# naver/deep-image-retrieval

Measured on AMD Instinct MI355X. Metric: images/sec descriptor extraction (resnet101-GeM, 1024x1024), higher is better.
Workload: dtype fp16p

## Files before the change

### deep-image-retrieval_amd/csrc/conv_igemm.hip

```cpp
#include "dir_common.h"
#include "conv_device.h"
#include "conv_igemm.h"

#include <stdlib.h>
#include <string.h>
#include <algorithm>

namespace dir {

template <class DT, int BM, int BN, int WGM, int WGN, int NST, int BK, bool CIN16, bool SPLITK>
__global__ void __launch_bounds__(64 * WGM * WGN) conv_igemm_kernel(const ConvArgs a) {
    static_assert(NST >= 2 && NST <= 8, "ring depth");
    static_assert((BK == 64 || BK == 32) && (!CIN16 || BK == 64), "K-step");
    constexpr int RB = BK * 2;
    constexpr int CPR = BK / 8;
    constexpr int KS = BK / 16;
    constexpr int NT = 64 * WGM * WGN;
    constexpr int TM = BM / WGM / 32;
    constexpr int TN = BN / WGN / 32;
    constexpr int NA = BM * CPR / NT;
    constexpr int NB = BN * CPR / NT;
    constexpr int LPS = NA + NB;
    static_assert(TM >= 1 && TN >= 1, "wave tile");
    static_assert(NA >= 1 && NB >= 1 && (BM * CPR) % NT == 0 && (BN * CPR) % NT == 0, "chunk split");
// ... 508 lines not shown
        (long)ceil_div(a.M, 64) * (a.Cout / 128) >= 96)
        return prev;
    return last;
}

int conv_pick_dual_variant(const ConvArgs& a, bool any_size) {
    const bool ok = a.x2 && a.R == 1 && a.S == 1 && a.stride == 1 && a.pad == 0 && a.H == a.OH && a.W == a.OW &&
                    a.Cin % 64 == 0 && a.Cin2 % 64 == 0 && a.res == nullptr && a.ksplit <= 1;
    if (!ok) return -1;
    {
        const int v = find_variant("64x256_wregd1x1");
        if (v >= 0 && !env().no_wregd && conv1x1_wregd_admissible(a) &&
            (any_size || (long)ceil_div(a.M, 64) * (a.Cout / 256) >= 1024))
            return v;
    }
    if (a.Cout % 256 != 0 || (!any_size && (long)ceil_div(a.M, 256) * (a.Cout / 256) < 192)) return -1;
    if (env().lc1x1) {
        const int vl = find_variant("256x256_lc1x1");
        if (vl >= 0 && conv1x1_lc_admissible(a)) return vl;
    }
    const int v = find_variant("256x256_persist1x1_x3");
    if (v < 0 || kVariants[v].launch_dual == nullptr) return -1;
    return v;
}

template <class DT>
__global__ void conv_splitk_finalize_kernel(const float* __restrict__ partial, const float* __restrict__ bias,
                                            const uint16_t* res, uint16_t* y,
                                            long total8, int Cout, long MC, int ksplit, int relu, int* ovf_flag) {
    const long i8 = (long)blockIdx.x * blockDim.x + threadIdx.x;
    if (i8 >= total8) return;
    const long o = i8 * 8;
    const int n = (int)(o % Cout);
    float v[8];
    const f32x4_t b0 = *(const DIR_GLOBAL f32x4_t*)(bias + n), b1 = *(const DIR_GLOBAL f32x4_t*)(bias + n + 4);
#pragma unroll
    for (int e = 0; e < 4; ++e) v[e] = b0[e], v[4 + e] = b1[e];
    for (int z = 0; z < ksplit; ++z) {
        const float* p = partial + (size_t)z * MC + o;
        const f32x4_t p0 = *(const DIR_GLOBAL f32x4_t*)p, p1 = *(const DIR_GLOBAL f32x4_t*)(p + 4);
#pragma unroll
        for (int e = 0; e < 4; ++e) v[e] += p0[e], v[4 + e] += p1[e];
    }
    if (res) {
        const u32x4_t rv = gload16(res + o);
#pragma unroll
        for (int e = 0; e < 4; ++e) {
            float lo, hi;
            DT::unpack(rv[e], lo, hi);
            v[2 * e] += lo;
            v[2 * e + 1] += hi;
        }
    }
    if (relu) relu8(v);
    const u32x4_t ov = pack8<DT>(v);
    gstore16(y + o, ov);
    Ovf<DT> ovf;
    ovf.see(ov);
    ovf.flush(ovf_flag);
}

size_t conv_splitk_bytes(const ConvArgs& a, int ksplit) {
    return ksplit > 1 ? (size_t)ksplit * a.M * a.Cout * sizeof(float) : 0;
}

int conv_splitk_factor(int v, const ConvArgs& a) {
    if (v < 0 || v >= kNumVariants || !kVariants[v].has_splitk || a.Cin == 16) return 1;
    const ConvVariant& cv = kVariants[v];
    const long tiles = (long)ceil_div(a.M, cv.BM) * (a.Cout / cv.BN);
    const int T = a.Ktot / cv.BK;
    if (tiles > 160 || T < 8) return 1;
    int s = (int)std::min<long>(std::min<long>(8, 512 / tiles), T / 4);
    while (s > 1 && conv_splitk_bytes(a, s) > kSplitKMaxBytes) --s;
    return s < 2 ? 1 : s;
}

int conv_launch(const ConvArgs& a, int dtype, int variant, hipStream_t stream) {
    if (a.Cout % 64 != 0) return fail(DIR_ERR_INVALID, "conv: Cout must be a multiple of 64");
    const bool cin16 = (a.Cin == 16);
    if (cin16) {
        if (a.R != 4 || a.S != 4 || a.stride != 1)
            return fail(DIR_ERR_INVALID, "conv: Cin == 16 is only the 4x4 s1 space-to-depth stem");
    } else if (a.Cin % 64 != 0) {
        return fail(DIR_ERR_INVALID, "conv: Cin must be a multiple of 64 (or 16 for the stem)");
    }
    if (a.R > 4 || a.S > 4) return fail(DIR_ERR_INVALID, "conv: filter larger than 4x4");
    if ((long)a.B * a.H * a.W * a.Cin >= (1L << 30) || (long)a.M * a.Cout >= (1L << 30) ||
        (long)a.Cout * a.Ktot >= (1L << 30))
        return fail(DIR_ERR_INVALID, "conv: tensor exceeds 2^31 bytes; lower the batch");
    if (((uintptr_t)a.x & 15) || ((uintptr_t)a.w & 15) || ((uintptr_t)a.y & 15) ||
        ((uintptr_t)a.res & 15) || ((uintptr_t)a.bias & 15))
        return fail(DIR_ERR_INVALID, "conv: tensors must be 16-byte aligned");
    if (dtype != DIR_BF16 && dtype != DIR_FP16) return fail(DIR_ERR_INVALID, "conv: bad dtype");
    if (a.x2) {
        if (variant < 0) variant = conv_pick_dual_variant(a);
        if (variant < 0 || variant >= kNumVariants || kVariants[variant].launch_dual == nullptr ||
            !kVariants[variant].admissible_dual(a) || a.R != 1 || a.S != 1 || a.stride != 1 || a.res || a.ksplit > 1 ||
            a.Cin2 % 64 != 0 || a.Ktot != a.Cin + a.Cin2 || ((uintptr_t)a.x2 & 15) ||
            (long)a.B * a.H2 * a.W2 * a.Cin2 >= (1L << 30))
            return fail(DIR_ERR_INVALID, "conv: no two-source form for this shape / variant");
        hipError_t e = kVariants[variant].launch_dual(a, dtype, stream);
        if (e != hipSuccess)
            return fail(DIR_ERR_HIP, std::string("conv launch ") + kVariants[variant].name + "/dual: " + hipGetErrorString(e));
        return DIR_OK;
    }
    if (variant < 0) variant = conv_pick_variant(a);
    if (!conv_variant_admissible(variant, a))
        return fail(DIR_ERR_INVALID, "conv: variant not admissible for this shape");
    const ConvVariant& cv = kVariants[variant];
    if (a.ksplit > 1) {
        if (!cv.has_splitk || cin16)
            return fail(DIR_ERR_INVALID, "conv: this variant has no split-K form");
        if (!a.partial || ((uintptr_t)a.partial & 15))
            return fail(DIR_ERR_INVALID, "conv: split-K needs a 16-byte aligned fp32 scratch buffer");
        if (a.ksplit > a.Ktot / cv.BK) return fail(DIR_ERR_INVALID, "conv: more K slices than K-steps");
    }
    hipError_t e = cv.launch(a, dtype, stream);
    if (e != hipSuccess)
        return fail(DIR_ERR_HIP, std::string("conv launch ") + cv.name + ": " + hipGetErrorString(e));
    if (a.ksplit > 1) {
        const long MC = (long)a.M * a.Cout, total8 = MC / 8;
        const dim3 grid((unsigned)((total8 + 255) / 256));
        if (dtype == DIR_BF16)
            hipLaunchKernelGGL(conv_splitk_finalize_kernel<BF16>, grid, dim3(256), 0, stream, a.partial, a.bias,
                               a.res, a.y, total8, a.Cout, MC, a.ksplit, a.relu, a.ovf);
        else
            hipLaunchKernelGGL(conv_splitk_finalize_kernel<FP16>, grid, dim3(256), 0, stream, a.partial, a.bias,
                               a.res, a.y, total8, a.Cout, MC, a.ksplit, a.relu, a.ovf);
        e = hipGetLastError();
        if (e != hipSuccess) return fail(DIR_ERR_HIP, std::string("conv split-K finalize: ") + hipGetErrorString(e));
    }
    return DIR_OK;
}

template <class DT>
__global__ void conv_naive_kernel(const ConvArgs a) {
    const long idx = (long)blockIdx.x * blockDim.x + threadIdx.x;
    if (idx >= (long)a.M * a.Cout) return;
    const int n = (int)(idx % a.Cout);
    const int m = (int)(idx / a.Cout);
    const int OHW = a.OH * a.OW;
    const int b = m / OHW, rem = m - b * OHW, oh = rem / a.OW, ow = rem - oh * a.OW;
    float acc = 0.f;
    for (int r = 0; r < a.R; ++r) {
        const int ih = oh * a.stride - a.pad + r;
        if ((unsigned)ih >= (unsigned)a.H) continue;
        for (int s = 0; s < a.S; ++s) {
            const int iw = ow * a.stride - a.pad + s;
            if ((unsigned)iw >= (unsigned)a.W) continue;
            const uint16_t* xp = a.x + ((size_t)(b * a.H + ih) * a.W + iw) * a.Cin;
            const uint16_t* wp = a.w + (size_t)n * a.Ktot + (r * a.S + s) * a.Cin;
            for (int c = 0; c < a.Cin; ++c) acc = fmaf(DT::to_f32(xp[c]), DT::to_f32(wp[c]), acc);
        }
    }
    float v = acc + a.bias[n];
    if (a.res) v += DT::to_f32(a.res[(size_t)m * a.Cout + n]);
    if (a.relu) v = fmaxf(v, 0.f);
    a.y[(size_t)m * a.Cout + n] = DT::from_f32(v);
}

int conv_launch_naive(const ConvArgs& a, int dtype, hipStream_t stream) {
    const long total = (long)a.M * a.Cout;
    const int threads = 256;
    const long blocks = (total + threads - 1) / threads;
    if (blocks >= (1L << 31)) return fail(DIR_ERR_INVALID, "naive conv: too many blocks");
    if (dtype == DIR_BF16)
        hipLaunchKernelGGL(conv_naive_kernel<BF16>, dim3((unsigned)blocks), dim3(threads), 0, stream, a);
// ... 9 lines not shown
```

### deep-image-retrieval_amd/csrc/conv_patchw.hip

```cpp
#include "dir_common.h"
#include "conv_device.h"
#include "conv_igemm.h"

#ifndef DIR_PATCHW_ABL
#define DIR_PATCHW_ABL 0
#endif

namespace dir {

template <class DT>
__global__ void __launch_bounds__(512) conv_patch3x3w_kernel(const ConvArgs a) {
    constexpr int TH = 16, TW = 32, PH = TH + 2, PW = TW + 2, PP = PH * PW;
    constexpr int NTH = 512, BN = 128;
    constexpr int NPL = (PP * 4 + NTH - 1) / NTH;
    constexpr int PLANE_BYTES = NPL * NTH * 16;
    constexpr int TN = 4, TMR = 2;
    constexpr int WSTAGE = 3 * BN * 64, NBW = WSTAGE / (NTH * 16);
    constexpr int NBW_X = (DIR_PATCHW_ABL & 16) ? 2 : 0;
    constexpr int NPL_X = (DIR_PATCHW_ABL & 32) ? 7 : 0;
    constexpr int NSTW = 3;
    constexpr int WOFF = 2 * PLANE_BYTES;
    constexpr int EROW = TN * 128 + 16;
    typedef typename DT::frag_t frag_t;
    static_assert(WOFF + NSTW * WSTAGE <= 160 * 1024 && NBW * NTH * 16 == WSTAGE, "LDS map");

    extern __shared__ __attribute__((aligned(16))) char smem[];

    const int tid = threadIdx.x;
    const int lane = tid & 63;
    const int wave = __builtin_amdgcn_readfirstlane(tid >> 6);
    const int lrow = lane & 31, lhi = lane >> 5;

    const int NQ = a.Cin / 32;
    const int NS = NQ * 3;
    const int tiles_n = a.Cout / BN;
    const int tiles_x = (a.OW + TW - 1) / TW;
    const int tiles_y = (a.OH + TH - 1) / TH;
    int wg = xcd_remap(blockIdx.x, gridDim.x);
    const int tile_n = wg % tiles_n;
    wg /= tiles_n;
    const int tx = wg % tiles_x;
    wg /= tiles_x;
    const int ty = wg % tiles_y;
    const int b = wg / tiles_y;
    const int oy0 = ty * TH, ox0 = tx * TW;

    const __amdgpu_buffer_rsrc_t rsrc_x = buffer_rsrc(a.x, a.x_bytes);
    const __amdgpu_buffer_rsrc_t rsrc_w = buffer_rsrc(a.w, a.w_bytes);

    uint32_t pvoff[NPL];
#pragma unroll
    for (int i = 0; i < NPL; ++i) {
        const int P = i * NTH + tid;
        const int p = P >> 2, pos = P & 3;
        const int py = p / PW, px = p - py * PW;
        const int iy = oy0 - 1 + py, ix = ox0 - 1 + px;
        const bool ok = p < PP && (unsigned)iy < (unsigned)a.H && (unsigned)ix < (unsigned)a.W;
        pvoff[i] = ok ? (uint32_t)((((b * a.H + iy) * a.W + ix) * a.Cin + ((pos ^ ((p >> 2) & 3)) << 3)) * 2) : kOOB;
    }
    auto issue_plane = [&](int q) {
        if (DIR_PATCHW_ABL & 64) return;
        char* dst = smem + (q & 1) * PLANE_BYTES;
#pragma unroll
        for (int i = 0; i < NPL; ++i) dma16(rsrc_x, dst + (i * NTH + wave * 64) * 16, pvoff[i], q * 64);
#pragma unroll
        for (int rep = 0; rep < NPL_X; ++rep)
#pragma unroll
            for (int i = 0; i < NPL; ++i) dma16(rsrc_x, dst + (i * NTH + wave * 64) * 16, pvoff[i], q * 64);
    };
    uint32_t wvoff[NBW];
#pragma unroll
    for (int i = 0; i < NBW; ++i) {
        const int L = i * NTH + tid;
        const int s = L >> 9, n = (L & 511) >> 2, pos = L & 3;
        wvoff[i] = (uint32_t)((((tile_n * BN + n) * 9 + s) * a.Cin + ((pos ^ ((n >> 2) & 3)) << 3)) * 2);
    }
    auto issue_w = [&](int sigma, int slot) {
        if (DIR_PATCHW_ABL & 64) return;
        const int q = sigma / 3, r = sigma - q * 3;
        char* dst = smem + WOFF + slot * WSTAGE;
#pragma unroll
        for (int i = 0; i < NBW; ++i) dma16(rsrc_w, dst + (i * NTH + wave * 64) * 16, wvoff[i], (r * 3 * a.Cin + q * 32) * 2);
#pragma unroll
        for (int i = 0; i < NBW_X; ++i)
            dma16(rsrc_w, dst + (i * NTH + wave * 64) * 16, wvoff[i], (((r + 1) % 3) * 3 * a.Cin + q * 32) * 2);
    };

    f32x16_t acc[TN][TMR];
#pragma unroll
    for (int i = 0; i < TN; ++i)
#pragma unroll
        for (int g = 0; g < 4; ++g) {
            const f32x4_t b4 = *(const DIR_GLOBAL f32x4_t*)(a.bias + tile_n * BN + i * 32 + 8 * g + 4 * lhi);
#pragma unroll
            for (int j = 0; j < TMR; ++j)
#pragma unroll
                for (int e = 0; e < 4; ++e) acc[i][j][4 * g + e] = b4[e];
        }

    int woffk[2];
#pragma unroll
    for (int kk = 0; kk < 2; ++kk) woffk[kk] = lrow * 64 + (((2 * kk + lhi) ^ ((lrow >> 2) & 3)) << 4);

    issue_plane(0);
    issue_w(0, 0);
    issue_w(1, 1);
    int q = 0, r = 0;
    int slot_c = 0;
    bool plane_before = false;
    for (int sigma = 0; sigma < NS; ++sigma) {
        if (((DIR_PATCHW_ABL & 4) && sigma == 0) || (DIR_PATCHW_ABL & 64)) {
        } else if (sigma + 1 >= NS) {
            asm volatile("s_waitcnt vmcnt(0)" ::: "memory");
        } else if (plane_before) {
            asm volatile("s_waitcnt vmcnt(%0)" ::"i"(NPL * (1 + NPL_X) + NBW + NBW_X) : "memory");
        } else {
            asm volatile("s_waitcnt vmcnt(%0)" ::"i"(NBW + NBW_X) : "memory");
        }
        ring_barrier();
        plane_before = false;
        if (r == 0 && q + 1 < NQ) {
            issue_plane(q + 1);
            plane_before = true;
        }
        if (sigma + 2 < NS) {
            int slot_n = slot_c + 2;
            if (slot_n >= NSTW) slot_n -= NSTW;
            issue_w(sigma + 2, slot_n);
        }
        const char* plane = smem + (q & 1) * PLANE_BYTES;
        const char* wst = smem + WOFF + slot_c * WSTAGE;
#pragma unroll
        for (int s = 0; s < ((DIR_PATCHW_ABL & 128) ? 0 : 3); ++s) {
            frag_t xf[TMR][2], wf[2][TN];
#pragma unroll
            for (int j = 0; j < TMR; ++j) {
                const int p = (wave * TMR + j + r) * PW + s + lrow;
                const int swz = (p >> 2) & 3;
#pragma unroll
                for (int kk = 0; kk < 2; ++kk) xf[j][kk] = *(const frag_t*)(plane + p * 64 + (((2 * kk + lhi) ^ swz) << 4));
            }
#pragma unroll
            for (int kk = 0; kk < 2; ++kk)
#pragma unroll
                for (int i = 0; i < TN; ++i) wf[kk][i] = *(const frag_t*)(wst + s * (BN * 64) + i * 2048 + woffk[kk]);
#pragma unroll
            for (int kk = 0; kk < 2; ++kk)
#pragma unroll
                for (int i = 0; i < TN; ++i)
#pragma unroll
                    for (int j = 0; j < TMR; ++j) {
                        if ((DIR_PATCHW_ABL & 8) && !(s == 0 || (s == 1 && kk == 0 && i < 3))) continue;
                        acc[i][j] = DT::mfma32(wf[kk][i], xf[j][kk], acc[i][j]);
                    }
        }
        asm volatile("s_waitcnt lgkmcnt(0)" ::: "memory");
        if (++slot_c == NSTW) slot_c = 0;
        if (++r == 3) {
            r = 0;
            ++q;
        }
    }
    __syncthreads();
    Ovf<DT> ovf;
    if (DIR_PATCHW_ABL & 2) {
        float sum = 0.f;
#pragma unroll
        for (int i = 0; i < TN; ++i)
#pragma unroll
            for (int j = 0; j < TMR; ++j)
#pragma unroll
                for (int e = 0; e < 16; ++e) sum += acc[i][j][e];
        if (sum == 1.2345678e30f) a.y[0] = 1;
        return;
    }

    char* ebase = smem + wave * (32 * EROW);
    constexpr int LPR = TN * 4, RPP = 64 / LPR, NPASS = 32 / RPP;
    const int ecol = (lane % LPR) * 8;
    const int erow = lane / LPR;
    const int ncol = tile_n * BN + ecol;
#pragma unroll
    for (int j = 0; j < TMR; ++j) {
#pragma unroll
        for (int i = 0; i < TN; ++i)
#pragma unroll
            for (int g = 0; g < 4; ++g) {
                f32x4_t v = {acc[i][j][4 * g + 0], acc[i][j][4 * g + 1], acc[i][j][4 * g + 2], acc[i][j][4 * g + 3]};
                *(f32x4_t*)(ebase + lrow * EROW + (i * 32 + 8 * g + 4 * lhi) * 4) = v;
            }
        wave_lds_sync();
        const int oy = oy0 + wave * TMR + j;
#pragma unroll
        for (int pass = 0; pass < NPASS; ++pass) {
            const int mrow = pass * RPP + erow;
            const f32x4_t f0 = *(const f32x4_t*)(ebase + mrow * EROW + ecol * 4);
            const f32x4_t f1 = *(const f32x4_t*)(ebase + mrow * EROW + ecol * 4 + 16);
            const int ox = ox0 + mrow;
            if (oy < a.OH && ox < a.OW) {
                float v[8] = {f0[0], f0[1], f0[2], f0[3], f1[0], f1[1], f1[2], f1[3]};
                const size_t o = ((size_t)(b * a.OH + oy) * a.OW + ox) * a.Cout + ncol;
                if (a.res) {
                    const u32x4_t rv = gload16(a.res + o);
#pragma unroll
                    for (int e = 0; e < 4; ++e) {
                        float lo, hi;
                        DT::unpack(rv[e], lo, hi);
                        v[2 * e] += lo;
                        v[2 * e + 1] += hi;
                    }
                }
                if (a.relu) relu8(v);
                const u32x4_t ov = pack8<DT>(v);
                if (!(DIR_PATCHW_ABL & 1) || ov[0] == 0x12345678u) gstore16(a.y + o, ov);
                ovf.see(ov);
            }
        }
        wave_lds_sync();
    }
    ovf.flush(a.ovf);
}

template <class DT>
__global__ void __launch_bounds__(768) conv_patch3x3w_lc_kernel(const ConvArgs a) {
    constexpr int TH = 16, TW = 32, PH = TH + 2, PW = TW + 2, PP = PH * PW;
    constexpr int NLD = 256, BN = 128;
    constexpr int NPL = (PP * 4 + NLD - 1) / NLD;
    constexpr int PLANE_BYTES = NPL * NLD * 16;
    constexpr int TN = 4, TMR = 2;
    constexpr int WSTAGE = 3 * BN * 64, NBW = WSTAGE / (NLD * 16);
    constexpr int NSTW = 3;
    constexpr int WOFF = 2 * PLANE_BYTES;
    constexpr int EROW = TN * 128 + 16;
    typedef typename DT::frag_t frag_t;
    static_assert(WOFF + NSTW * WSTAGE <= 160 * 1024 && NBW * NLD * 16 == WSTAGE, "LDS map");

    extern __shared__ __attribute__((aligned(16))) char smem[];

    const int tid = threadIdx.x;
    const int lane = tid & 63;
    const int wave = __builtin_amdgcn_readfirstlane(tid >> 6);
    const int lrow = lane & 31, lhi = lane >> 5;

    const int NQ = a.Cin / 32;
    const int NS = NQ * 3;
    const int tiles_n = a.Cout / BN;
    const int tiles_x = (a.OW + TW - 1) / TW;
    const int tiles_y = (a.OH + TH - 1) / TH;
    int wg = xcd_remap(blockIdx.x, gridDim.x);
    const int tile_n = wg % tiles_n;
    wg /= tiles_n;
    const int tx = wg % tiles_x;
    wg /= tiles_x;
    const int ty = wg % tiles_y;
    const int b = wg / tiles_y;
    const int oy0 = ty * TH, ox0 = tx * TW;

    if (wave >= 8) {
        const int lt = tid - 512;
        const int lw = wave - 8;
        const __amdgpu_buffer_rsrc_t rsrc_x = buffer_rsrc(a.x, a.x_bytes);
        uint32_t pvoff[NPL];
#pragma unroll
        for (int i = 0; i < NPL; ++i) {
            const int P = i * NLD + lt;
            const int p = P >> 2, pos = P & 3;
            const int py = p / PW, px = p - py * PW;
            const int iy = oy0 - 1 + py, ix = ox0 - 1 + px;
            const bool ok = p < PP && (unsigned)iy < (unsigned)a.H && (unsigned)ix < (unsigned)a.W;
            pvoff[i] = ok ? (uint32_t)((((b * a.H + iy) * a.W + ix) * a.Cin + ((pos ^ ((p >> 2) & 3)) << 3)) * 2) : kOOB;
        }
        const bool packed = a.w_pw != nullptr;
        const __amdgpu_buffer_rsrc_t rsrc_wp = buffer_rsrc(packed ? a.w_pw : a.w, a.w_bytes);
        uint32_t wvoff[NBW];
#pragma unroll
        for (int i = 0; i < NBW; ++i) {
            const int L = i * NLD + lt;
            const int s = L >> 9, n = (L & 511) >> 2, pos = L & 3;
            wvoff[i] = packed ? (uint32_t)(L * 16) : (uint32_t)((((tile_n * BN + n) * 9 + s) * a.Cin + ((pos ^ ((n >> 2) & 3)) << 3)) * 2);
        }
        auto issue_plane = [&](int q) {
            char* dst = smem + (q & 1) * PLANE_BYTES;
#pragma unroll
            for (int i = 0; i < NPL; ++i) dma16(rsrc_x, dst + (i * NLD + lw * 64) * 16, pvoff[i], q * 64);
        };
        auto issue_w = [&](int sigma, int slot) {
            const int q = sigma / 3, r = sigma - q * 3;
            char* dst = smem + WOFF + slot * WSTAGE;
            const int soff = packed ? (tile_n * NS + sigma) * WSTAGE : (r * 3 * a.Cin + q * 32) * 2;
#pragma unroll
            for (int i = 0; i < NBW; ++i) dma16(rsrc_wp, dst + (i * NLD + lw * 64) * 16, wvoff[i], soff);
        };
        issue_plane(0);
        issue_w(0, 0);
        if (NS > 1) issue_w(1, 1);
        int q = 0, r = 0, slot_c = 0;
        bool plane_before = false;
        for (int sigma = 0; sigma < NS; ++sigma) {
            if (sigma + 1 >= NS) {
                asm volatile("s_waitcnt vmcnt(0)" ::: "memory");
            } else if (plane_before) {
                asm volatile("s_waitcnt vmcnt(%0)" ::"i"(NPL + NBW) : "memory");
            } else {
                asm volatile("s_waitcnt vmcnt(%0)" ::"i"(NBW) : "memory");
            }
            ring_barrier();
            plane_before = false;
            if (r == 0 && q + 1 < NQ) {
                issue_plane(q + 1);
                plane_before = true;
            }
            if (sigma + 2 < NS) {
                int slot_n = slot_c + 2;
                if (slot_n >= NSTW) slot_n -= NSTW;
                issue_w(sigma + 2, slot_n);
            }
            if (++slot_c == NSTW) slot_c = 0;
            if (++r == 3) {
                r = 0;
                ++q;
            }
        }
        ring_barrier();
        return;
    }

    f32x16_t acc[TN][TMR];
#pragma unroll
    for (int i = 0; i < TN; ++i)
#pragma unroll
        for (int g = 0; g < 4; ++g) {
            const f32x4_t b4 = *(const DIR_GLOBAL f32x4_t*)(a.bias + tile_n * BN + i * 32 + 8 * g + 4 * lhi);
#pragma unroll
            for (int j = 0; j < TMR; ++j)
#pragma unroll
                for (int e = 0; e < 4; ++e) acc[i][j][4 * g + e] = b4[e];
        }
    int woffk[2];
#pragma unroll
    for (int kk = 0; kk < 2; ++kk) woffk[kk] = lrow * 64 + (((2 * kk + lhi) ^ ((lrow >> 2) & 3)) << 4);
    asm volatile("s_waitcnt vmcnt(0)" ::: "memory");

    int q = 0, r = 0, slot_c = 0;
    for (int sigma = 0; sigma < NS; ++sigma) {
        ring_barrier();
        const char* plane = smem + (q & 1) * PLANE_BYTES;
        const char* wst = smem + WOFF + slot_c * WSTAGE;
#pragma unroll
        for (int s = 0; s < 3; ++s) {
#pragma unroll
            for (int kk = 0; kk < 2; ++kk) {
                frag_t xf[TMR], wf[TN];
#pragma unroll
                for (int j = 0; j < TMR; ++j) {
                    const int p = (wave * TMR + j + r) * PW + s + lrow;
                    xf[j] = *(const frag_t*)(plane + p * 64 + (((2 * kk + lhi) ^ ((p >> 2) & 3)) << 4));
                }
#pragma unroll
                for (int i = 0; i < TN; ++i) wf[i] = *(const frag_t*)(wst + s * (BN * 64) + i * 2048 + woffk[kk]);
#pragma unroll
                for (int j = 0; j < TMR; ++j)
#pragma unroll
                    for (int i = 0; i < TN; ++i) acc[i][j] = DT::mfma32(wf[i], xf[j], acc[i][j]);
            }
        }
        asm volatile("s_waitcnt lgkmcnt(0)" ::: "memory");
        if (++slot_c == NSTW) slot_c = 0;
        if (++r == 3) {
            r = 0;
            ++q;
        }
    }
    ring_barrier();
    Ovf<DT> ovf;
    char* ebase = smem + wave * (32 * EROW);
    constexpr int LPR = TN * 4, RPP = 64 / LPR, NPASS = 32 / RPP;
    const int ecol = (lane % LPR) * 8;
    const int erow = lane / LPR;
    const int ncol = tile_n * BN + ecol;
#pragma unroll
    for (int j = 0; j < TMR; ++j) {
#pragma unroll
        for (int i = 0; i < TN; ++i)
#pragma unroll
            for (int g = 0; g < 4; ++g) {
                f32x4_t v = {acc[i][j][4 * g + 0], acc[i][j][4 * g + 1], acc[i][j][4 * g + 2], acc[i][j][4 * g + 3]};
                *(f32x4_t*)(ebase + lrow * EROW + (i * 32 + 8 * g + 4 * lhi) * 4) = v;
            }
        wave_lds_sync();
        const int oy = oy0 + wave * TMR + j;
#pragma unroll
        for (int pass = 0; pass < NPASS; ++pass) {
            const int mrow = pass * RPP + erow;
            const f32x4_t f0 = *(const f32x4_t*)(ebase + mrow * EROW + ecol * 4);
            const f32x4_t f1 = *(const f32x4_t*)(ebase + mrow * EROW + ecol * 4 + 16);
            const int ox = ox0 + mrow;
            if (oy < a.OH && ox < a.OW) {
                float v[8] = {f0[0], f0[1], f0[2], f0[3], f1[0], f1[1], f1[2], f1[3]};
                const size_t o = ((size_t)(b * a.OH + oy) * a.OW + ox) * a.Cout + ncol;
                if (a.res) {
                    const u32x4_t rv = gload16(a.res + o);
#pragma unroll
                    for (int e = 0; e < 4; ++e) {
                        float lo, hi;
                        DT::unpack(rv[e], lo, hi);
                        v[2 * e] += lo;
                        v[2 * e + 1] += hi;
                    }
                }
                if (a.relu) relu8(v);
                const u32x4_t ov = pack8<DT>(v);
                gstore16(a.y + o, ov);
                ovf.see(ov);
            }
        }
        wave_lds_sync();
    }
    ovf.flush(a.ovf);
}

bool conv_patch3x3w_admissible(const ConvArgs& a) {
    return a.R == 3 && a.S == 3 && a.stride == 1 && a.pad == 1 && a.H == a.OH && a.W == a.OW && a.Cin % 32 == 0 &&
           a.Cin >= 64 && a.Cout % 128 == 0 && (size_t)a.B * a.H * a.W * a.Cin * 2 < (1ull << 31) &&
           (size_t)a.Cout * a.Ktot * 2 < (1ull << 31);
}

__global__ void __launch_bounds__(256) pack_patchw_kernel(const uint16_t* w, uint16_t* out, int Cout, int Cin) {
    const int NQ = Cin / 32;
    const long pieces = (long)Cout * 9 * Cin / 8;
    for (long i = (long)blockIdx.x * 256 + threadIdx.x; i < pieces; i += (long)gridDim.x * 256) {
        const int L = (int)(i % 1536);
        long t = i / 1536;
        const int r = (int)(t % 3);
        t /= 3;
        const int q = (int)(t % NQ);
        const int tn = (int)(t / NQ);
        const int s = L >> 9, n = (L & 511) >> 2, pos = L & 3;
        const size_t src = ((size_t)((tn * 128 + n) * 9 + r * 3 + s)) * Cin + q * 32 + ((pos ^ ((n >> 2) & 3)) << 3);
        gstore16(out + i * 8, gload16(w + src));
    }
}

hipError_t conv_patch3x3w_pack(const uint16_t* w, uint16_t* out, int Cout, int Cin, hipStream_t stream) {
    const long pieces = (long)Cout * 9 * Cin / 8;
    const int grid = (int)((pieces + 255) / 256 < 1024 ? (pieces + 255) / 256 : 1024);
    hipLaunchKernelGGL(pack_patchw_kernel, dim3(grid), dim3(256), 0, stream, w, out, Cout, Cin);
    return hipGetLastError();
}

template <class DT>
static hipError_t launch_patch_w(const ConvArgs& a, hipStream_t stream) {
    constexpr int LDS = 2 * 5 * 512 * 16 + 3 * 3 * 128 * 64;
    static_assert(LDS <= 160 * 1024 && LDS >= 8 * 32 * (4 * 128 + 16), "LDS map (the staging area aliases it)");
    ConvArgs b = a;
    conv_fill_extents(b);
    const long blocks = (long)a.B * ((a.OH + 15) / 16) * ((a.OW + 31) / 32) * (a.Cout / 128);
    if (!env().no_patchw_lc) {
        void* scratch = nullptr;
        if (!b.w_pw && env().patchw_pack) {
            if (hipError_t e = hipMallocAsync(&scratch, b.w_bytes, stream); e != hipSuccess) return e;
            if (hipError_t e = conv_patch3x3w_pack(a.w, (uint16_t*)scratch, a.Cout, a.Cin, stream); e != hipSuccess) {
                (void)hipFreeAsync(scratch, stream);
                return e;
            }
            b.w_pw = (const uint16_t*)scratch;
        }
        auto kern = conv_patch3x3w_lc_kernel<DT>;
        static std::atomic<uint64_t> attr_lc{0};
        if (hipError_t e = ensure_dynamic_lds((const void*)kern, LDS, attr_lc); e != hipSuccess) return e;
        hipLaunchKernelGGL(kern, dim3((unsigned)blocks), dim3(768), LDS, stream, b);
        hipError_t e = hipGetLastError();
        if (scratch) {
            const hipError_t f = hipFreeAsync(scratch, stream);
            if (e == hipSuccess) e = f;
        }
        return e;
    }
    auto kern = conv_patch3x3w_kernel<DT>;
    static std::atomic<uint64_t> attr_done{0};
    if (hipError_t e = ensure_dynamic_lds((const void*)kern, LDS, attr_done); e != hipSuccess) return e;
    hipLaunchKernelGGL(kern, dim3((unsigned)blocks), dim3(512), LDS, stream, b);
    return hipGetLastError();
}

hipError_t conv_patch3x3w_launch(const ConvArgs& a, int dtype, hipStream_t stream) {
    return dtype == DIR_BF16 ? launch_patch_w<BF16>(a, stream) : launch_patch_w<FP16>(a, stream);
}

}
```

### deep-image-retrieval_amd/csrc/dir_common.h

```cpp
#pragma once
#include <hip/hip_runtime.h>
#include <stdint.h>
#include <string.h>
#include <atomic>
#include <string>

#include "../../include/dir_engine.h"

namespace dir {

typedef __attribute__((ext_vector_type(8))) __bf16 bf16x8_t;
typedef __attribute__((ext_vector_type(8))) _Float16 f16x8_t;
typedef __attribute__((ext_vector_type(16))) float f32x16_t;
typedef __attribute__((ext_vector_type(4))) float f32x4_t;
typedef __attribute__((ext_vector_type(4))) uint32_t u32x4_t;
typedef __attribute__((ext_vector_type(2))) uint32_t u32x2_t;
typedef __attribute__((ext_vector_type(2))) float f32x2_t;
typedef __attribute__((ext_vector_type(2))) __bf16 bf16x2_t;
typedef __attribute__((ext_vector_type(2))) _Float16 f16x2_t;

#define DIR_GLOBAL __attribute__((address_space(1)))
#define DIR_LDS __attribute__((address_space(3)))

void set_error(const std::string& msg);
int fail(int code, const std::string& msg);

#define DIR_HIP_CHECK(expr)                                                                \
    do {                                                                                   \
        hipError_t _e = (expr);                                                            \
        if (_e != hipSuccess)                                                              \
            return ::dir::fail(DIR_ERR_HIP, std::string(#expr) + ": " + hipGetErrorString(_e)); \
    } while (0)

struct Env {
    bool c3c1_off = false, c3c1_force = false;
    bool no_ds_seam = false, no_dual = false;
    bool rev_conv1 = false, rev_conv3 = false;
    bool unfused_stem = false, stem_v1 = false;
    bool no_patchlc = false, no_wreg = false, no_patchw = false, no_x3 = false, no_patchs = false;
    bool patchw_pack = false, no_patchw_pack = false;
    bool small_k2 = false;
    bool no_patchs2 = false;
    bool x3_k2048 = false;
    bool lc1x1 = false;
    bool no_c3c1lc = false;
    bool no_smallmap = false;
    bool no_wregd = false;
    bool no_patchw_lc = false;
    bool no_xcdmap = false;
    bool no_pair_patch = false, pair_acts = false;
    int pair_stages = 1;
    bool sim_v1 = false, sim_exact = false;
    bool experiments = false;
    bool no_inplace = false;
    bool no_stem_u8 = false;
    bool stem_pair_old = false;
    bool stem_u8_prep = false;
    bool stem_u8_wg8 = false;
    int stem_u8_seg = 0;
};
const Env& env();
void reload_env();

__host__ __device__ inline uint16_t f32_to_bf16_bits(float f) {
    uint32_t u;
    memcpy(&u, &f, 4);
    if ((u & 0x7fffffffu) > 0x7f800000u) return (uint16_t)((u >> 16) | 0x40);
    u += 0x7fffu + ((u >> 16) & 1u);
    return (uint16_t)(u >> 16);
}
__host__ __device__ inline float bf16_bits_to_f32(uint16_t h) {
    uint32_t u = ((uint32_t)h) << 16;
    float f;
    memcpy(&f, &u, 4);
    return f;
}
__host__ __device__ inline uint16_t f32_to_f16_bits(float f) {
    _Float16 h = (_Float16)f;
    uint16_t b;
    memcpy(&b, &h, 2);
    return b;
}
__host__ __device__ inline float f16_bits_to_f32(uint16_t b) {
    _Float16 h;
    memcpy(&h, &b, 2);
    return (float)h;
}

struct BF16 {
    typedef bf16x8_t frag_t;
    static constexpr int kDtype = DIR_BF16;
    __host__ __device__ static inline float to_f32(uint16_t b) { return bf16_bits_to_f32(b); }
    __host__ __device__ static inline uint16_t from_f32(float f) { return f32_to_bf16_bits(f); }
    __device__ static inline f32x16_t mfma32(frag_t a, frag_t b, f32x16_t c) {
        return __builtin_amdgcn_mfma_f32_32x32x16_bf16(a, b, c, 0, 0, 0);
    }
    __device__ static inline void unpack(uint32_t w, float& lo, float& hi) {
        lo = __builtin_bit_cast(float, w << 16);
        hi = __builtin_bit_cast(float, w & 0xffff0000u);
    }
    __device__ static inline uint32_t pack(float lo, float hi) {
        const f32x2_t v = {lo, hi};
        return __builtin_bit_cast(uint32_t, __builtin_convertvector(v, bf16x2_t));
    }
};
struct FP16 {
    typedef f16x8_t frag_t;
    static constexpr int kDtype = DIR_FP16;
    __host__ __device__ static inline float to_f32(uint16_t b) { return f16_bits_to_f32(b); }
    __host__ __device__ static inline uint16_t from_f32(float f) { return f32_to_f16_bits(f); }
    __device__ static inline f32x16_t mfma32(frag_t a, frag_t b, f32x16_t c) {
        return __builtin_amdgcn_mfma_f32_32x32x16_f16(a, b, c, 0, 0, 0);
    }
    __device__ static inline void unpack(uint32_t w, float& lo, float& hi) {
        const f32x2_t v = __builtin_convertvector(__builtin_bit_cast(f16x2_t, w), f32x2_t);
        lo = v[0];
        hi = v[1];
    }
    __device__ static inline uint32_t pack(float lo, float hi) {
        const f32x2_t v = {lo, hi};
        return __builtin_bit_cast(uint32_t, __builtin_convertvector(v, f16x2_t));
    }
};

template <class DT>
__device__ inline void unpack2(uint32_t w, float& lo, float& hi) {
    lo = DT::to_f32((uint16_t)(w & 0xffffu));
    hi = DT::to_f32((uint16_t)(w >> 16));
}
template <class DT>
__device__ inline uint32_t pack2(float lo, float hi) {
    return (uint32_t)DT::from_f32(lo) | ((uint32_t)DT::from_f32(hi) << 16);
}

__device__ inline u32x4_t gload16(const void* p) {
    return *(const DIR_GLOBAL u32x4_t*)p;
}
__device__ inline void gstore16(void* p, u32x4_t v) {
    *(DIR_GLOBAL u32x4_t*)p = v;
}

typedef __attribute__((ext_vector_type(2))) uint16_t u16x2_t;
template <class DT>
struct Ovf {
    uint32_t m = 0;
    __device__ inline void see(uint32_t w) {
        if constexpr (DT::kDtype == DIR_FP16) {
            uint32_t t;
            asm("v_and_b32 %1, 0x7fff7fff, %2\n\tv_pk_max_u16 %0, %0, %1" : "+v"(m), "=&v"(t) : "v"(w));
        }
    }
    __device__ inline void see(const u32x4_t& v) {
#pragma unroll
        for (int e = 0; e < 4; ++e) see(v[e]);
    }
    __device__ inline void see(const u32x2_t& v) {
        see(v[0]);
        see(v[1]);
    }
    __device__ inline void flush(int* flag) const {
        if constexpr (DT::kDtype == DIR_FP16) {
            if (flag && ((m + 0x04000400u) & 0x80008000u)) atomicOr(flag, 1);
        }
    }
};

__device__ __forceinline__ void ring_barrier() {
#ifndef DIR_EXP_NO_RING_FENCE
    __builtin_amdgcn_sched_barrier(0);
#endif
    __builtin_amdgcn_s_barrier();
#ifndef DIR_EXP_NO_RING_FENCE
    __builtin_amdgcn_sched_barrier(0);
#endif
}

__device__ inline int xcd_remap(int bid, int nwg) {
    const int q = nwg >> 3, r = nwg & 7, xcd = bid & 7;
    const int start = xcd < r ? xcd * (q + 1) : r * (q + 1) + (xcd - r) * q;
    return start + (bid >> 3);
}

inline int ceil_div(int a, int b) { return (a + b - 1) / b; }

inline int cu_count() {
    static std::atomic<int> cached[64];
    int dev = 0;
    if (hipGetDevice(&dev) != hipSuccess) return 256;
    int n = cached[dev & 63].load(std::memory_order_relaxed);
    if (n > 0) return n;
    hipDeviceProp_t prop;
    n = hipGetDeviceProperties(&prop, dev) == hipSuccess && prop.multiProcessorCount > 0 ? prop.multiProcessorCount : 256;
    cached[dev & 63].store(n, std::memory_order_relaxed);
    return n;
}
// ... 14 lines not shown
```

Baseline: 2471.

## Switch patch 3x3 conv kernels to 16x16x32 MFMA with new LDS swizzle

```diff
diff --git a/deep-image-retrieval_amd/csrc/conv_igemm.hip b/deep-image-retrieval_amd/csrc/conv_igemm.hip
--- a/deep-image-retrieval_amd/csrc/conv_igemm.hip
+++ b/deep-image-retrieval_amd/csrc/conv_igemm.hip
@@ -614,7 +614,9 @@
         if (a.R != 4 || a.S != 4 || a.stride != 1)
             return fail(DIR_ERR_INVALID, "conv: Cin == 16 is only the 4x4 s1 space-to-depth stem");
     } else if (a.Cin % 64 != 0) {
-        return fail(DIR_ERR_INVALID, "conv: Cin must be a multiple of 64 (or 16 for the stem)");
+        const bool planes32 = variant >= 0 && variant < kNumVariants && kVariants[variant].launch == conv_patch3x3w_launch &&
+                              a.Cin % 32 == 0 && a.ksplit <= 1 && !a.x2;
+        if (!planes32) return fail(DIR_ERR_INVALID, "conv: Cin must be a multiple of 64 (or 16 for the stem)");
     }
     if (a.R > 4 || a.S > 4) return fail(DIR_ERR_INVALID, "conv: filter larger than 4x4");
     if ((long)a.B * a.H * a.W * a.Cin >= (1L << 30) || (long)a.M * a.Cout >= (1L << 30) ||
diff --git a/deep-image-retrieval_amd/csrc/conv_patchw.hip b/deep-image-retrieval_amd/csrc/conv_patchw.hip
--- a/deep-image-retrieval_amd/csrc/conv_patchw.hip
+++ b/deep-image-retrieval_amd/csrc/conv_patchw.hip
@@ -1,12 +1,100 @@
 #include "dir_common.h"
 #include "conv_device.h"
 #include "conv_igemm.h"
+#include "patchw_layout.h"
 
 #ifndef DIR_PATCHW_ABL
 #define DIR_PATCHW_ABL 0
 #endif
 
 namespace dir {
+
+typedef f32x4_t PatchwAcc[8][4];
+
+__device__ __forceinline__ void patchw_bias_init(PatchwAcc& acc, const float* bias, int tile_n, int lane) {
+#pragma unroll
+    for (int i = 0; i < 8; ++i) {
+        const f32x4_t b4 = *(const DIR_GLOBAL f32x4_t*)(bias + tile_n * 128 + patchw::stage_channel(i, lane));
+#pragma unroll
+        for (int t = 0; t < 4; ++t) acc[i][t] = b4;
+    }
+}
+
+template <class DT>
+__device__ __forceinline__ void patchw_stage(PatchwAcc& acc, const char* plane, const char* wst, int wave, int r, int lane) {
+    typedef typename DT::frag_t frag_t;
+    const char* wl = wst + patchw::frag_off(0, lane);
+    frag_t xf[4], wf[24];
+    __builtin_amdgcn_sched_barrier(0);
+#pragma unroll
+    for (int k = 0; k < 2; ++k) wf[k] = *(const frag_t*)(wl + patchw::wfrag_off(k >> 3, k & 7, 0));
+#pragma unroll
+    for (int k = 0; k < 24; k += 2) {
+        const int s = k >> 3, i = k & 7;
+        if (i == 0) {
+#pragma unroll
+            for (int t = 0; t < 4; ++t) xf[t] = *(const frag_t*)(plane + patchw::xfrag_off(wave, t, r, s, lane));
+        }
+        if (k + 2 < 24) {
+#pragma unroll
+            for (int d = 2; d < 4; ++d) wf[k + d] = *(const frag_t*)(wl + patchw::wfrag_off((k + d) >> 3, (k + d) & 7, 0));
+        }
+        __builtin_amdgcn_sched_barrier(0);
+#pragma unroll
+        for (int t = 0; t < 4; ++t)
+#pragma unroll
+            for (int d = 0; d < 2; ++d) acc[i + d][t] = DT::mfma16(wf[k + d], xf[t], acc[i + d][t]);
+        __builtin_amdgcn_sched_barrier(0);
+    }
+}
+
+template <class DT>
+__device__ __forceinline__ void patchw_epilogue(const ConvArgs& a, PatchwAcc& acc, char* smem, int wave, int lane, int b, int oy0, int ox0,
+                                                int tile_n) {
+    constexpr int EROW = patchw::kERow;
+    Ovf<DT> ovf;
+    char* ebase = smem + wave * (32 * EROW);
+    constexpr int LPR = 16, RPP = 64 / LPR, NPASS = 32 / RPP;
+    const int ecol = (lane % LPR) * 8;
+    const int erow = lane / LPR;
+    const int ncol = tile_n * 128 + ecol;
+#pragma unroll
+    for (int j = 0; j < 2; ++j) {
+#pragma unroll
+        for (int i = 0; i < 8; ++i)
+#pragma unroll
+            for (int h = 0; h < 2; ++h) *(f32x4_t*)(ebase + patchw::stage_off(i, h, lane)) = acc[i][2 * j + h];
+        wave_lds_sync();
+        const int oy = oy0 + wave * 2 + j;
+#pragma unroll
+        for (int pass = 0; pass < NPASS; ++pass) {
+            const int mrow = pass * RPP + erow;
+            const f32x4_t f0 = *(const f32x4_t*)(ebase + mrow * EROW + ecol * 4);
+            const f32x4_t f1 = *(const f32x4_t*)(ebase + mrow * EROW + ecol * 4 + 16);
+            const int ox = ox0 + mrow;
+            if (oy < a.OH && ox < a.OW) {
+                float v[8] = {f0[0], f0[1], f0[2], f0[3], f1[0], f1[1], f1[2], f1[3]};
+                const size_t o = ((size_t)(b * a.OH + oy) * a.OW + ox) * a.Cout + ncol;
+                if (a.res) {
+                    const u32x4_t rv = gload16(a.res + o);
+#pragma unroll
+                    for (int e = 0; e < 4; ++e) {
+                        float lo, hi;
+                        DT::unpack(rv[e], lo, hi);
+                        v[2 * e] += lo;
+                        v[2 * e + 1] += hi;
+                    }
+                }
+                if (a.relu) relu8(v);
+                const u32x4_t ov = pack8<DT>(v);
+                if (!(DIR_PATCHW_ABL & 1) || ov[0] == 0x12345678u) gstore16(a.y + o, ov);
+                ovf.see(ov);
+            }
+        }
+        wave_lds_sync();
+    }
+    ovf.flush(a.ovf);
+}
 
 template <class DT>
 __global__ void __launch_bounds__(512) conv_patch3x3w_kernel(const ConvArgs a) {
@@ -14,22 +102,16 @@
     constexpr int NTH = 512, BN = 128;
     constexpr int NPL = (PP * 4 + NTH - 1) / NTH;
     constexpr int PLANE_BYTES = NPL * NTH * 16;
-    constexpr int TN = 4, TMR = 2;
     constexpr int WSTAGE = 3 * BN * 64, NBW = WSTAGE / (NTH * 16);
-    constexpr int NBW_X = (DIR_PATCHW_ABL & 16) ? 2 : 0;
-    constexpr int NPL_X = (DIR_PATCHW_ABL & 32) ? 7 : 0;
     constexpr int NSTW = 3;
     constexpr int WOFF = 2 * PLANE_BYTES;
-    constexpr int EROW = TN * 128 + 16;
-    typedef typename DT::frag_t frag_t;
-    static_assert(WOFF + NSTW * WSTAGE <= 160 * 1024 && NBW * NTH * 16 == WSTAGE, "LDS map");
+    static_assert(WOFF + NSTW * WSTAGE <= 160 * 1024 && NBW * NTH * 16 == WSTAGE && PW == 34, "LDS map");
 
     extern __shared__ __attribute__((aligned(16))) char smem[];
 
     const int tid = threadIdx.x;
     const int lane = tid & 63;
     const int wave = __builtin_amdgcn_readfirstlane(tid >> 6);
-    const int lrow = lane & 31, lhi = lane >> 5;
 
     const int NQ = a.Cin / 32;
     const int NS = NQ * 3;
@@ -52,28 +134,24 @@
 #pragma unroll
     for (int i = 0; i < NPL; ++i) {
         const int P = i * NTH + tid;
-        const int p = P >> 2, pos = P & 3;
+        const int p = P >> 2;
         const int py = p / PW, px = p - py * PW;
         const int iy = oy0 - 1 + py, ix = ox0 - 1 + px;
         const bool ok = p < PP && (unsigned)iy < (unsigned)a.H && (unsigned)ix < (unsigned)a.W;
-        pvoff[i] = ok ? (uint32_t)((((b * a.H + iy) * a.W + ix) * a.Cin + ((pos ^ ((p >> 2) & 3)) << 3)) * 2) : kOOB;
+        pvoff[i] = ok ? (uint32_t)((((b * a.H + iy) * a.W + ix) * a.Cin + (patchw::piece_chunk(P) << 3)) * 2) : kOOB;
     }
     auto issue_plane = [&](int q) {
         if (DIR_PATCHW_ABL & 64) return;
         char* dst = smem + (q & 1) * PLANE_BYTES;
 #pragma unroll
         for (int i = 0; i < NPL; ++i) dma16(rsrc_x, dst + (i * NTH + wave * 64) * 16, pvoff[i], q * 64);
-#pragma unroll
-        for (int rep = 0; rep < NPL_X; ++rep)
-#pragma unroll
-            for (int i = 0; i < NPL; ++i) dma16(rsrc_x, dst + (i * NTH + wave * 64) * 16, pvoff[i], q * 64);
     };
     uint32_t wvoff[NBW];
 #pragma unroll
     for (int i = 0; i < NBW; ++i) {
         const int L = i * NTH + tid;
-        const int s = L >> 9, n = (L & 511) >> 2, pos = L & 3;
-        wvoff[i] = (uint32_t)((((tile_n * BN + n) * 9 + s) * a.Cin + ((pos ^ ((n >> 2) & 3)) << 3)) * 2);
+        const int s = L >> 9, n = (L & 511) >> 2;
+        wvoff[i] = (uint32_t)((((tile_n * BN + n) * 9 + s) * a.Cin + (patchw::piece_chunk(L) << 3)) * 2);
     }
     auto issue_w = [&](int sigma, int slot) {
         if (DIR_PATCHW_ABL & 64) return;
@@ -81,26 +159,10 @@
         char* dst = smem + WOFF + slot * WSTAGE;
 #pragma unroll
         for (int i = 0; i < NBW; ++i) dma16(rsrc_w, dst + (i * NTH + wave * 64) * 16, wvoff[i], (r * 3 * a.Cin + q * 32) * 2);
-#pragma unroll
-        for (int i = 0; i < NBW_X; ++i)
-            dma16(rsrc_w, dst + (i * NTH + wave * 64) * 16, wvoff[i], (((r + 1) % 3) * 3 * a.Cin + q * 32) * 2);
     };
 
-    f32x16_t acc[TN][TMR];
-#pragma unroll
-    for (int i = 0; i < TN; ++i)
-#pragma unroll
-        for (int g = 0; g < 4; ++g) {
-            const f32x4_t b4 = *(const DIR_GLOBAL f32x4_t*)(a.bias + tile_n * BN + i * 32 + 8 * g + 4 * lhi);
-#pragma unroll
-            for (int j = 0; j < TMR; ++j)
-#pragma unroll
-                for (int e = 0; e < 4; ++e) acc[i][j][4 * g + e] = b4[e];
-        }
-
-    int woffk[2];
-#pragma unroll
-    for (int kk = 0; kk < 2; ++kk) woffk[kk] = lrow * 64 + (((2 * kk + lhi) ^ ((lrow >> 2) & 3)) << 4);
+    PatchwAcc acc;
+    patchw_bias_init(acc, a.bias, tile_n, lane);
 
     issue_plane(0);
     issue_w(0, 0);
@@ -113,9 +175,9 @@
         } else if (sigma + 1 >= NS) {
             asm volatile("s_waitcnt vmcnt(0)" ::: "memory");
         } else if (plane_before) {
-            asm volatile("s_waitcnt vmcnt(%0)" ::"i"(NPL * (1 + NPL_X) + NBW + NBW_X) : "memory");
+            asm volatile("s_waitcnt vmcnt(%0)" ::"i"(NPL + NBW) : "memory");
         } else {
-            asm volatile("s_waitcnt vmcnt(%0)" ::"i"(NBW + NBW_X) : "memory");
+            asm volatile("s_waitcnt vmcnt(%0)" ::"i"(NBW) : "memory");
         }
         ring_barrier();
         plane_before = false;
@@ -128,32 +190,7 @@
             if (slot_n >= NSTW) slot_n -= NSTW;
             issue_w(sigma + 2, slot_n);
         }
-        const char* plane = smem + (q & 1) * PLANE_BYTES;
-        const char* wst = smem + WOFF + slot_c * WSTAGE;
-#pragma unroll
-        for (int s = 0; s < ((DIR_PATCHW_ABL & 128) ? 0 : 3); ++s) {
-            frag_t xf[TMR][2], wf[2][TN];
-#pragma unroll
-            for (int j = 0; j < TMR; ++j) {
-                const int p = (wave * TMR + j + r) * PW + s + lrow;
-                const int swz = (p >> 2) & 3;
-#pragma unroll
-                for (int kk = 0; kk < 2; ++kk) xf[j][kk] = *(const frag_t*)(plane + p * 64 + (((2 * kk + lhi) ^ swz) << 4));
-            }
-#pragma unroll
-            for (int kk = 0; kk < 2; ++kk)
-#pragma unroll
-                for (int i = 0; i < TN; ++i) wf[kk][i] = *(const frag_t*)(wst + s * (BN * 64) + i * 2048 + woffk[kk]);
-#pragma unroll
-            for (int kk = 0; kk < 2; ++kk)
-#pragma unroll
-                for (int i = 0; i < TN; ++i)
-#pragma unroll
-                    for (int j = 0; j < TMR; ++j) {
-                        if ((DIR_PATCHW_ABL & 8) && !(s == 0 || (s == 1 && kk == 0 && i < 3))) continue;
-                        acc[i][j] = DT::mfma32(wf[kk][i], xf[j][kk], acc[i][j]);
-                    }
-        }
+        if (!(DIR_PATCHW_ABL & 128)) patchw_stage<DT>(acc, smem + (q & 1) * PLANE_BYTES, smem + WOFF + slot_c * WSTAGE, wave, r, lane);
         asm volatile("s_waitcnt lgkmcnt(0)" ::: "memory");
         if (++slot_c == NSTW) slot_c = 0;
         if (++r == 3) {
@@ -162,63 +199,18 @@
         }
     }
     __syncthreads();
-    Ovf<DT> ovf;
     if (DIR_PATCHW_ABL & 2) {
         float sum = 0.f;
 #pragma unroll
-        for (int i = 0; i < TN; ++i)
-#pragma unroll
-            for (int j = 0; j < TMR; ++j)
-#pragma unroll
-                for (int e = 0; e < 16; ++e) sum += acc[i][j][e];
+        for (int i = 0; i < 8; ++i)
+#pragma unroll
+            for (int t = 0; t < 4; ++t)
+#pragma unroll
+                for (int e = 0; e < 4; ++e) sum += acc[i][t][e];
         if (sum == 1.2345678e30f) a.y[0] = 1;
         return;
     }
-
-    char* ebase = smem + wave * (32 * EROW);
-    constexpr int LPR = TN * 4, RPP = 64 / LPR, NPASS = 32 / RPP;
-    const int ecol = (lane % LPR) * 8;
-    const int erow = lane / LPR;
-    const int ncol = tile_n * BN + ecol;
-#pragma unroll
-    for (int j = 0; j < TMR; ++j) {
-#pragma unroll
-        for (int i = 0; i < TN; ++i)
-#pragma unroll
-            for (int g = 0; g < 4; ++g) {
-                f32x4_t v = {acc[i][j][4 * g + 0], acc[i][j][4 * g + 1], acc[i][j][4 * g + 2], acc[i][j][4 * g + 3]};
-                *(f32x4_t*)(ebase + lrow * EROW + (i * 32 + 8 * g + 4 * lhi) * 4) = v;
-            }
-        wave_lds_sync();
-        const int oy = oy0 + wave * TMR + j;
-#pragma unroll
-        for (int pass = 0; pass < NPASS; ++pass) {
-            const int mrow = pass * RPP + erow;
-            const f32x4_t f0 = *(const f32x4_t*)(ebase + mrow * EROW + ecol * 4);
-            const f32x4_t f1 = *(const f32x4_t*)(ebase + mrow * EROW + ecol * 4 + 16);
-            const int ox = ox0 + mrow;
-            if (oy < a.OH && ox < a.OW) {
-                float v[8] = {f0[0], f0[1], f0[2], f0[3], f1[0], f1[1], f1[2], f1[3]};
-                const size_t o = ((size_t)(b * a.OH + oy) * a.OW + ox) * a.Cout + ncol;
-                if (a.res) {
-                    const u32x4_t rv = gload16(a.res + o);
-#pragma unroll
-                    for (int e = 0; e < 4; ++e) {
-                        float lo, hi;
-                        DT::unpack(rv[e], lo, hi);
-                        v[2 * e] += lo;
-                        v[2 * e + 1] += hi;
-                    }
-                }
-                if (a.relu) relu8(v);
-                const u32x4_t ov = pack8<DT>(v);
-                if (!(DIR_PATCHW_ABL & 1) || ov[0] == 0x12345678u) gstore16(a.y + o, ov);
-                ovf.see(ov);
-            }
-        }
-        wave_lds_sync();
-    }
-    ovf.flush(a.ovf);
+    patchw_epilogue<DT>(a, acc, smem, wave, lane, b, oy0, ox0, tile_n);
 }
 
 template <class DT>
@@ -227,20 +219,16 @@
     constexpr int NLD = 256, BN = 128;
     constexpr int NPL = (PP * 4 + NLD - 1) / NLD;
     constexpr int PLANE_BYTES = NPL * NLD * 16;
-    constexpr int TN = 4, TMR = 2;
     constexpr int WSTAGE = 3 * BN * 64, NBW = WSTAGE / (NLD * 16);
     constexpr int NSTW = 3;
     constexpr int WOFF = 2 * PLANE_BYTES;
-    constexpr int EROW = TN * 128 + 16;
-    typedef typename DT::frag_t frag_t;
-    static_assert(WOFF + NSTW * WSTAGE <= 160 * 1024 && NBW * NLD * 16 == WSTAGE, "LDS map");
+    static_assert(WOFF + NSTW * WSTAGE <= 160 * 1024 && NBW * NLD * 16 == WSTAGE && PW == 34, "LDS map");
 
     extern __shared__ __attribute__((aligned(16))) char smem[];
 
     const int tid = threadIdx.x;
     const int lane = tid & 63;
     const int wave = __builtin_amdgcn_readfirstlane(tid >> 6);
-    const int lrow = lane & 31, lhi = lane >> 5;
 
     const int NQ = a.Cin / 32;
     const int NS = NQ * 3;
@@ -264,11 +252,11 @@
 #pragma unroll
         for (int i = 0; i < NPL; ++i) {
             const int P = i * NLD + lt;
-            const int p = P >> 2, pos = P & 3;
+            const int p = P >> 2;
             const int py = p / PW, px = p - py * PW;
             const int iy = oy0 - 1 + py, ix = ox0 - 1 + px;
             const bool ok = p < PP && (unsigned)iy < (unsigned)a.H && (unsigned)ix < (unsigned)a.W;
-            pvoff[i] = ok ? (uint32_t)((((b * a.H + iy) * a.W + ix) * a.Cin + ((pos ^ ((p >> 2) & 3)) << 3)) * 2) : kOOB;
+            pvoff[i] = ok ? (uint32_t)((((b * a.H + iy) * a.W + ix) * a.Cin + (patchw::piece_chunk(P) << 3)) * 2) : kOOB;
         }
         const bool packed = a.w_pw != nullptr;
         const __amdgpu_buffer_rsrc_t rsrc_wp = buffer_rsrc(packed ? a.w_pw : a.w, a.w_bytes);
@@ -276,8 +264,8 @@
 #pragma unroll
         for (int i = 0; i < NBW; ++i) {
             const int L = i * NLD + lt;
-            const int s = L >> 9, n = (L & 511) >> 2, pos = L & 3;
-            wvoff[i] = packed ? (uint32_t)(L * 16) : (uint32_t)((((tile_n * BN + n) * 9 + s) * a.Cin + ((pos ^ ((n >> 2) & 3)) << 3)) * 2);
+            const int s = L >> 9, n = (L & 511) >> 2;
+            wvoff[i] = packed ? (uint32_t)(L * 16) : (uint32_t)((((tile_n * BN + n) * 9 + s) * a.Cin + (patchw::piece_chunk(L) << 3)) * 2);
         }
         auto issue_plane = [&](int q) {
             char* dst = smem + (q & 1) * PLANE_BYTES;
@@ -325,45 +313,14 @@
         return;
     }
 
-    f32x16_t acc[TN][TMR];
-#pragma unroll
-    for (int i = 0; i < TN; ++i)
-#pragma unroll
-        for (int g = 0; g < 4; ++g) {
-            const f32x4_t b4 = *(const DIR_GLOBAL f32x4_t*)(a.bias + tile_n * BN + i * 32 + 8 * g + 4 * lhi);
-#pragma unroll
-            for (int j = 0; j < TMR; ++j)
-#pragma unroll
-                for (int e = 0; e < 4; ++e) acc[i][j][4 * g + e] = b4[e];
-        }
-    int woffk[2];
-#pragma unroll
-    for (int kk = 0; kk < 2; ++kk) woffk[kk] = lrow * 64 + (((2 * kk + lhi) ^ ((lrow >> 2) & 3)) << 4);
+    PatchwAcc acc;
+    patchw_bias_init(acc, a.bias, tile_n, lane);
     asm volatile("s_waitcnt vmcnt(0)" ::: "memory");
 
     int q = 0, r = 0, slot_c = 0;
     for (int sigma = 0; sigma < NS; ++sigma) {
         ring_barrier();
-        const char* plane = smem + (q & 1) * PLANE_BYTES;
-        const char* wst = smem + WOFF + slot_c * WSTAGE;
-#pragma unroll
-        for (int s = 0; s < 3; ++s) {
-#pragma unroll
-            for (int kk = 0; kk < 2; ++kk) {
-                frag_t xf[TMR], wf[TN];
-#pragma unroll
-                for (int j = 0; j < TMR; ++j) {
-                    const int p = (wave * TMR + j + r) * PW + s + lrow;
-                    xf[j] = *(const frag_t*)(plane + p * 64 + (((2 * kk + lhi) ^ ((p >> 2) & 3)) << 4));
-                }
-#pragma unroll
-                for (int i = 0; i < TN; ++i) wf[i] = *(const frag_t*)(wst + s * (BN * 64) + i * 2048 + woffk[kk]);
-#pragma unroll
-                for (int j = 0; j < TMR; ++j)
-#pragma unroll
-                    for (int i = 0; i < TN; ++i) acc[i][j] = DT::mfma32(wf[i], xf[j], acc[i][j]);
-            }
-        }
+        patchw_stage<DT>(acc, smem + (q & 1) * PLANE_BYTES, smem + WOFF + slot_c * WSTAGE, wave, r, lane);
         asm volatile("s_waitcnt lgkmcnt(0)" ::: "memory");
         if (++slot_c == NSTW) slot_c = 0;
         if (++r == 3) {
@@ -372,51 +329,7 @@
         }
     }
     ring_barrier();
-    Ovf<DT> ovf;
-    char* ebase = smem + wave * (32 * EROW);
-    constexpr int LPR = TN * 4, RPP = 64 / LPR, NPASS = 32 / RPP;
-    const int ecol = (lane % LPR) * 8;
-    const int erow = lane / LPR;
-    const int ncol = tile_n * BN + ecol;
-#pragma unroll
-    for (int j = 0; j < TMR; ++j) {
-#pragma unroll
-        for (int i = 0; i < TN; ++i)
-#pragma unroll
-            for (int g = 0; g < 4; ++g) {
-                f32x4_t v = {acc[i][j][4 * g + 0], acc[i][j][4 * g + 1], acc[i][j][4 * g + 2], acc[i][j][4 * g + 3]};
-                *(f32x4_t*)(ebase + lrow * EROW + (i * 32 + 8 * g + 4 * lhi) * 4) = v;
-            }
-        wave_lds_sync();
-        const int oy = oy0 + wave * TMR + j;
-#pragma unroll
-        for (int pass = 0; pass < NPASS; ++pass) {
-            const int mrow = pass * RPP + erow;
-            const f32x4_t f0 = *(const f32x4_t*)(ebase + mrow * EROW + ecol * 4);
-            const f32x4_t f1 = *(const f32x4_t*)(ebase + mrow * EROW + ecol * 4 + 16);
-            const int ox = ox0 + mrow;
-            if (oy < a.OH && ox < a.OW) {
-                float v[8] = {f0[0], f0[1], f0[2], f0[3], f1[0], f1[1], f1[2], f1[3]};
-                const size_t o = ((size_t)(b * a.OH + oy) * a.OW + ox) * a.Cout + ncol;
-                if (a.res) {
-                    const u32x4_t rv = gload16(a.res + o);
-#pragma unroll
-                    for (int e = 0; e < 4; ++e) {
-                        float lo, hi;
-                        DT::unpack(rv[e], lo, hi);
-                        v[2 * e] += lo;
-                        v[2 * e + 1] += hi;
-                    }
-                }
-                if (a.relu) relu8(v);
-                const u32x4_t ov = pack8<DT>(v);
-                gstore16(a.y + o, ov);
-                ovf.see(ov);
-            }
-        }
-        wave_lds_sync();
-    }
-    ovf.flush(a.ovf);
+    patchw_epilogue<DT>(a, acc, smem, wave, lane, b, oy0, ox0, tile_n);
 }
 
 bool conv_patch3x3w_admissible(const ConvArgs& a) {
@@ -435,8 +348,8 @@
         t /= 3;
         const int q = (int)(t % NQ);
         const int tn = (int)(t / NQ);
-        const int s = L >> 9, n = (L & 511) >> 2, pos = L & 3;
-        const size_t src = ((size_t)((tn * 128 + n) * 9 + r * 3 + s)) * Cin + q * 32 + ((pos ^ ((n >> 2) & 3)) << 3);
+        const int s = L >> 9, n = (L & 511) >> 2;
+        const size_t src = ((size_t)((tn * 128 + n) * 9 + r * 3 + s)) * Cin + q * 32 + (patchw::piece_chunk(L) << 3);
         gstore16(out + i * 8, gload16(w + src));
     }
 }
diff --git a/deep-image-retrieval_amd/csrc/dir_common.h b/deep-image-retrieval_amd/csrc/dir_common.h
--- a/deep-image-retrieval_amd/csrc/dir_common.h
+++ b/deep-image-retrieval_amd/csrc/dir_common.h
@@ -95,6 +95,9 @@
     __device__ static inline f32x16_t mfma32(frag_t a, frag_t b, f32x16_t c) {
         return __builtin_amdgcn_mfma_f32_32x32x16_bf16(a, b, c, 0, 0, 0);
     }
+    __device__ static inline f32x4_t mfma16(frag_t a, frag_t b, f32x4_t c) {
+        return __builtin_amdgcn_mfma_f32_16x16x32_bf16(a, b, c, 0, 0, 0);
+    }
     __device__ static inline void unpack(uint32_t w, float& lo, float& hi) {
         lo = __builtin_bit_cast(float, w << 16);
         hi = __builtin_bit_cast(float, w & 0xffff0000u);
@@ -111,6 +114,9 @@
     __host__ __device__ static inline uint16_t from_f32(float f) { return f32_to_f16_bits(f); }
     __device__ static inline f32x16_t mfma32(frag_t a, frag_t b, f32x16_t c) {
         return __builtin_amdgcn_mfma_f32_32x32x16_f16(a, b, c, 0, 0, 0);
+    }
+    __device__ static inline f32x4_t mfma16(frag_t a, frag_t b, f32x4_t c) {
+        return __builtin_amdgcn_mfma_f32_16x16x32_f16(a, b, c, 0, 0, 0);
     }
     __device__ static inline void unpack(uint32_t w, float& lo, float& hi) {
         const f32x2_t v = __builtin_convertvector(__builtin_bit_cast(f16x2_t, w), f32x2_t);
diff --git a/deep-image-retrieval_amd/csrc/patchw_layout.h b/deep-image-retrieval_amd/csrc/patchw_layout.h
--- /dev/null
+++ b/deep-image-retrieval_amd/csrc/patchw_layout.h
@@ -0,0 +1,34 @@
+#pragma once
+
+#if defined(__HIPCC__) || defined(__CUDACC__)
+#define PATCHW_HD __host__ __device__
+#else
+#define PATCHW_HD
+#endif
+
+namespace dir {
+namespace patchw {
+
+constexpr int kRowBytes = 64;
+constexpr int kERow = 4 * 128 + 16;
+
+PATCHW_HD constexpr int swz(int row) { return ((row >> 2) & 1) << 1; }
+
+PATCHW_HD constexpr int piece_off(int row, int chunk) { return row * kRowBytes + ((chunk ^ swz(row)) << 4); }
+
+PATCHW_HD constexpr int piece_chunk(int P) { return (P & 3) ^ swz(P >> 2); }
+
+PATCHW_HD constexpr int frag_off(int row0, int lane) { return piece_off(row0 + (lane & 15), lane >> 4); }
+
+PATCHW_HD constexpr int wfrag_off(int s, int i, int lane) { return s * (128 * kRowBytes) + frag_off(i * 16, lane); }
+PATCHW_HD constexpr int patch_row0(int wave, int t, int r, int s) { return (wave * 2 + (t >> 1) + r) * 34 + s + (t & 1) * 16; }
+PATCHW_HD constexpr int xfrag_off(int wave, int t, int r, int s, int lane) {
+    return frag_off(patch_row0(wave, t & 2, r, s), lane) + (t & 1) * 16 * kRowBytes;
+}
+
+PATCHW_HD constexpr int stage_pixel(int t, int lane) { return (t & 1) * 16 + (lane & 15); }
+PATCHW_HD constexpr int stage_channel(int i, int lane) { return i * 16 + 4 * (lane >> 4); }
+PATCHW_HD constexpr int stage_off(int i, int t, int lane) { return stage_pixel(t, lane) * kERow + stage_channel(i, lane) * 4; }
+
+}
+}
```

After: 2458. About the same (-0.5%).
